# WestlyPark/StyleRenderer

Hardware: AMD Instinct MI355X
Metric: generator fwd+bwd images/sec at 256^2 (higher is better)
Workload: dtype f32

## Files before the change

stylerenderer_amd/build.py:

```python
import os
import subprocess
import sys

HERE = os.path.dirname(os.path.abspath(__file__))
CSRC = os.path.join(HERE, "csrc")
LIB = os.path.join(HERE, "libstylerenderer_hip.so")
OBJ = os.path.join(HERE, "csrc", "_obj")

ARCH = "gfx950"
COMMON = ["--offload-arch=" + ARCH, "-O3", "-std=c++17", "-fPIC", "-Wno-unused-result",
          "-fhip-fp32-correctly-rounded-divide-sqrt"]
EXACT = ["-ffp-contract=off"]
NOSLP = ["-fno-slp-vectorize"]

SOURCES = [
    ("capi.hip", EXACT),
    ("fused_bias_act.hip", EXACT),
    ("upfirdn2d.hip", EXACT + NOSLP),
    ("rasterize.hip", EXACT),
    ("fused_elem.hip", EXACT),
    ("weight_prep.hip", EXACT),
    ("style_linear.hip", EXACT),
    ("bank_mm.hip", EXACT),
    ("mesh.hip", EXACT),
    ("lpips.hip", EXACT),
    ("conv_mfma.hip", []),
    ("conv_wino.hip", []),
    ("conv_wgrad_wino.hip", []),
    ("conv_wgrad_mfma.hip", []),
    ("conv_wgrad_bf16x3.hip", []),
    ("conv_s2_bf16x3.hip", []),
    ("conv_generic.hip", []),
    ("conv1x1_gemm.hip", []),
]


def _hipcc():
    for c in (os.environ.get("HIPCC"), "/opt/rocm/bin/hipcc", "hipcc"):
        if c and (os.path.isabs(c) and os.path.exists(c) or not os.path.isabs(c)):
            return c
    return "hipcc"


def _deps(src):
    deps = [src, os.path.join(CSRC, "common.h"),
            os.path.join(HERE, "..", "include", "stylerenderer_amd.h"), os.path.abspath(__file__)]
    deps += [os.path.join(CSRC, f) for f in os.listdir(CSRC) if f.endswith(".h")]
    return max(os.path.getmtime(d) for d in deps if os.path.exists(d))


def build_library(force=False, verbose=False):
    os.makedirs(OBJ, exist_ok=True)
    hipcc = _hipcc()
    objs, rebuilt = [], False
    procs = []
    for name, extra in SOURCES:
        src = os.path.join(CSRC, name)
        obj = os.path.join(OBJ, name.replace(".hip", ".o"))
        objs.append(obj)
        if force or not os.path.exists(obj) or os.path.getmtime(obj) < _deps(src):
            cmd = [hipcc] + COMMON + extra + ["-c", src, "-o", obj]
            if verbose:
                print(" ".join(cmd))
            procs.append((name, subprocess.Popen(cmd, stdout=subprocess.PIPE, stderr=subprocess.STDOUT)))
            rebuilt = True
    for name, p in procs:
        out, _ = p.communicate()
        if p.returncode != 0:
            sys.stderr.write(out.decode(errors="replace"))
            raise RuntimeError("hipcc failed on %s" % name)
        if verbose and out:
            sys.stdout.write(out.decode(errors="replace"))
    if rebuilt or not os.path.exists(LIB):
        cmd = [hipcc, "--offload-arch=" + ARCH, "-shared", "-fPIC", "-o", LIB] + objs
        if verbose:
            print(" ".join(cmd))
        subprocess.check_call(cmd)
    return LIB


if __name__ == "__main__":
    print(build_library(force="-f" in sys.argv, verbose=True))
```

stylerenderer_amd/csrc/conv_mfma.hip:

```cpp
#include "common.h"
#include "conv1x1_gemm.h"
#include "conv_s2_bf16x3.h"
#include "conv_wgrad_bf16x3.h"
#include "conv_wino.h"

#include <cstdlib>

namespace {

typedef float f32x16 __attribute__((ext_vector_type(16)));
typedef const void __attribute__((address_space(1)))* gptr_t;
typedef void __attribute__((address_space(3)))* lptr_t;

constexpr int BN = 128;
constexpr int BM = 128;

__device__ __attribute__((aligned(16))) const float g_zero_line[4] = {0.f, 0.f, 0.f, 0.f};
__device__ __attribute__((aligned(16))) const float g_ones_line[4] = {1.f, 1.f, 1.f, 1.f};

struct ConvParams {
    const float* in;
    const float* wt;
    const float* iscale;
    const float* oscale;
    const float* obias;
    float* out;
    int B, C, N, ldw;
    int IH, IW;
    int GH, GW;
    int gy_base, gx_base;
    int OH, OW;
    int osy, osx, ooy, oox;
    int dy0, dx0;
    int wmap[9];
    int tiles_x, tiles_y, tiles_b, tiles_n;
    float* partial;
    int64_t partial_floats;
    int ks, c_per_slice;
    int tap_first, tap_step, tap_count;
};

template <int IS, int TY, int TX, int PW, int PH, int PB, bool V4, bool TAP9 = false>
struct Geo {
    static constexpr bool ROT = V4 && IS == 2;
    static constexpr int NT = TY * TX;
    static constexpr int KC = NT >= 9 ? 4 : (NT >= 4 ? 8 : 16);
    static constexpr int EH = (PH - 1) * IS + TY;
    static constexpr int EW = (PW - 1) * IS + TX;
    static constexpr int LEAD = (V4 && !ROT) ? (TAP9 ? 4 : (TX > 1 ? 3 : 0)) : 0;
    static constexpr int EWP = ROT ? (EW + 3 + 3) / 4 * 4
                                   : (V4 ? (LEAD + EW + 3) / 4 * 4 : EW + ((EW % 2 == 0) ? 1 : 0));
    static constexpr int PLANE = PB * EH * EWP;
    static constexpr int W_FLOATS = NT * KC * BN;
    static constexpr int W_INSTR = W_FLOATS / 256;
    static constexpr int IMG_INSTR = V4 ? (KC * PLANE + 255) / 256 : 0;
    static constexpr int ST_INSTR = V4 ? (KC * PB + 63) / 64 : 0;
    static constexpr int IN_FLOATS = KC * PLANE + KC * PB;
    static constexpr int IN_INSTR = V4 ? IMG_INSTR + ST_INSTR : (IN_FLOATS + 63) / 64;
    static constexpr int S_BASE = V4 ? W_FLOATS + IMG_INSTR * 256 : W_FLOATS + KC * PLANE;
    static constexpr int BUF = V4 ? S_BASE + ST_INSTR * 64 : W_FLOATS + IN_INSTR * 64;
    static constexpr int W_PER_WAVE = (W_INSTR + 3) / 4;
    static constexpr int IN_PER_WAVE = (IN_INSTR + 3) / 4;
    static constexpr int LDS_BYTES = 2 * BUF * 4;
};

template <int IS, int TY, int TX, int PW, int PH, int PB, bool V4, bool FAST, bool TAP9 = false>
__global__ __launch_bounds__(256) void k_conv_mfma(const ConvParams p) {
    using G = Geo<IS, TY, TX, PW, PH, PB, V4, TAP9>;
    static_assert(PW * PH * PB == BM, "patch must hold 128 pixels");
    static_assert(!TAP9 || (IS == 1 && TY == 1 && TX == 1), "tap-split mode is a shifted 1x1 convolution");
    extern __shared__ __attribute__((aligned(16))) float smem[];

    const int nwg = gridDim.x;
    int bid = blockIdx.x;
    {
        const int q = nwg / SR_NUM_XCD, r = nwg % SR_NUM_XCD, xcd = bid % SR_NUM_XCD;
        bid = (xcd < r ? xcd * (q + 1) : r * (q + 1) + (xcd - r) * q) + bid / SR_NUM_XCD;
    }
    int tap = 0, g_dy0 = p.dy0, g_dx0 = p.dx0, g_gh = p.GH, g_gw = p.GW, g_ooy = p.ooy, g_oox = p.oox, g_slab = p.wmap[0];
    int tap_local = 0;
    if (TAP9) {
        tap_local = bid % p.tap_count;
        bid /= p.tap_count;
        tap = p.tap_first + tap_local * p.tap_step;
        const int ky = tap / 3, kx = tap - 3 * ky;
        g_dy0 = -(ky >> 1); g_dx0 = -(kx >> 1);
        g_ooy = ky & 1; g_oox = kx & 1;
        g_gh = min(g_ooy ? p.IH : p.IH + 1, p.GH); g_gw = min(g_oox ? p.IW : p.IW + 1, p.GW);
        g_slab = tap;
    }
    const int n_t = bid % p.tiles_n;
    bid /= p.tiles_n;
    const int tx_i = bid % p.tiles_x;
    bid /= p.tiles_x;
    const int ty_i = bid % p.tiles_y;
    bid /= p.tiles_y;
    const int tb_i = bid % p.tiles_b;
    const int slice = bid / p.tiles_b;
    const int c_beg = slice * p.c_per_slice;
    const int c_end = min(p.C, c_beg + p.c_per_slice);
    const int n0 = n_t * BN, gy0 = p.gy_base + ty_i * PH, gx0 = p.gx_base + tx_i * PW, b0 = tb_i * PB;
    const int iy0 = gy0 * IS + g_dy0, ix0 = gx0 * IS + g_dx0;

    const int tid = threadIdx.x, lane = tid & 63;
    const int wave = __builtin_amdgcn_readfirstlane(tid >> 6);
    const int half = lane >> 5, l31 = lane & 31;
    const int wco = wave & 1, wpx = wave >> 1;

    int a_off[2], b_off[2], s_off[2];
    int b_rot[2][4];
#pragma unroll
    for (int t = 0; t < 2; ++t) {
        a_off[t] = half * BN + wco * 64 + t * 32 + l31;
        const int m = wpx * 64 + t * 32 + l31;
        const int px = m % PW, py = (m / PW) % PH, pb = m / (PW * PH);
        b_off[t] = G::W_FLOATS + half * G::PLANE + (pb * G::EH + py * IS) * G::EWP + px * IS + G::LEAD +
                   ((TAP9 && V4) ? g_dx0 : 0);
        s_off[t] = G::S_BASE + pb * G::KC + half;
        const int l0 = half + iy0 + py * IS + ix0;
#pragma unroll
        for (int k = 0; k < 4; ++k) b_rot[t][k] = b_off[t] + ((l0 + k) & 3);
    }

    int w_src[G::W_PER_WAVE];
    int w_cl[G::W_PER_WAVE];
#pragma unroll
    for (int i = 0; i < G::W_PER_WAVE; ++i) {
        const int j = wave + 4 * i;
        const int row = 2 * j + half;
        const int t = row / G::KC, c = row % G::KC;
        const int col = min(n0 + l31 * 4, p.ldw - 4);
        w_cl[i] = (j < G::W_INSTR) ? c : -1;
        int slab = 0;
#pragma unroll
        for (int k = 0; k < G::NT; ++k)
            if (t == k) slab = p.wmap[k];
        if (TAP9) slab = g_slab;
        w_src[i] = (slab * p.C + c) * p.ldw + col;
    }
    int i_src[G::IN_PER_WAVE];
    int i_cl[G::IN_PER_WAVE];
#pragma unroll
    for (int i = 0; i < G::IN_PER_WAVE; ++i) {
        const int j = wave + 4 * i;
        int src = -1, c = 0, pb = 0;
        if (V4) {
            const int f = (j * 64 + lane) * 4;
            if (j < G::IMG_INSTR && f < G::KC * G::PLANE) {
                c = f / G::PLANE;
                const int q = f % G::PLANE;
                const int cola = q % G::EWP, r = (q / G::EWP) % G::EH;
                pb = q / (G::EWP * G::EH);
                const int gy = iy0 + r;
                int gx = ((TAP9 && V4) ? gx0 : ix0) - G::LEAD + cola;
                bool ok = gy >= 0 && gy < p.IH && b0 + pb < p.B;
                if (G::ROT) {
                    gx = ix0 - ((c * (p.IH * p.IW) + gy * p.IW + ix0) & 3) + cola;
                } else {
                    ok = ok && gx >= 0 && gx + 3 < p.IW;
                }
                if (ok) src = (pb * p.C + c) * p.IH * p.IW + gy * p.IW + gx;
            } else if (j >= G::IMG_INSTR && j < G::IN_INSTR) {
                const int e = (j - G::IMG_INSTR) * 64 + lane;
                if (e < G::KC * PB) {
                    pb = e / G::KC;
                    c = e % G::KC;
                    src = -2;
                }
            }
        } else {
            const int f = j * 64 + lane;
            if (j < G::IN_INSTR && f < G::KC * G::PLANE) {
                c = f / G::PLANE;
                const int q = f % G::PLANE;
                const int colp = q % G::EWP, r = (q / G::EWP) % G::EH;
                pb = q / (G::EWP * G::EH);
                const int gy = iy0 + r, gx = ix0 + colp;
                if (colp < G::EW && gy >= 0 && gy < p.IH && gx >= 0 && gx < p.IW && b0 + pb < p.B)
                    src = (pb * p.C + c) * p.IH * p.IW + gy * p.IW + gx;
            } else if (j < G::IN_INSTR && f < G::IN_FLOATS) {
                const int e = f - G::KC * G::PLANE;
                pb = e / G::KC;
                c = e % G::KC;
                src = -2;
            }
        }
        i_src[i] = src;
        i_cl[i] = c | (pb << 8);
    }
    const float* in_base = p.in + (int64_t)b0 * p.C * p.IH * p.IW;
    const int plane_in = p.IH * p.IW;

    const char* f_wp[G::W_PER_WAVE];
    const char* f_ip[G::IN_PER_WAVE];
    unsigned f_is[G::IN_PER_WAVE];
    if (FAST) {
#pragma unroll
        for (int i = 0; i < G::W_PER_WAVE; ++i) f_wp[i] = reinterpret_cast<const char*>(p.wt + w_src[i]);
#pragma unroll
        for (int i = 0; i < G::IN_PER_WAVE; ++i) {
            const int c = i_cl[i] & 255, pb = i_cl[i] >> 8;
            const char* ptr = reinterpret_cast<const char*>(g_zero_line);
            unsigned str = 0;
            if (i_src[i] >= 0) {
                ptr = reinterpret_cast<const char*>(in_base + i_src[i]);
                str = (unsigned)plane_in * 4u;
            } else if (i_src[i] == -2) {
                const bool ok = p.iscale && b0 + pb < p.B;
                ptr = ok ? reinterpret_cast<const char*>(p.iscale + (int64_t)(b0 + pb) * p.C + c)
                         : reinterpret_cast<const char*>(g_ones_line);
                str = ok ? 4u : 0u;
            }
            f_ip[i] = ptr;
            f_is[i] = str;
        }
    }
    const unsigned w_chunk_stride = (unsigned)p.ldw * 4u;

    auto dma = [&](int c0, int buf) {
        float* dst = smem + buf * G::BUF;
        if (FAST) {
#pragma unroll
            for (int i = 0; i < G::W_PER_WAVE; ++i) {
                const int j = wave + 4 * i;
                if (j < G::W_INSTR)
                    __builtin_amdgcn_global_load_lds((gptr_t)(f_wp[i] + (uint64_t)(unsigned)c0 * w_chunk_stride),
                                                     (lptr_t)(dst + j * 256), 16, 0, 0);
            }
#pragma unroll
            for (int i = 0; i < G::IN_PER_WAVE; ++i) {
                const int j = wave + 4 * i;
                if (j < G::IN_INSTR) {
                    const char* src = f_ip[i] + (uint64_t)(unsigned)c0 * f_is[i];
                    if (V4 && j < G::IMG_INSTR)
                        __builtin_amdgcn_global_load_lds((gptr_t)src, (lptr_t)(dst + G::W_FLOATS + j * 256), 16, 0, 0);
                    else if (V4)
                        __builtin_amdgcn_global_load_lds((gptr_t)src,
                                                         (lptr_t)(dst + G::S_BASE + (j - G::IMG_INSTR) * 64), 4, 0, 0);
                    else
                        __builtin_amdgcn_global_load_lds((gptr_t)src, (lptr_t)(dst + G::W_FLOATS + j * 64), 4, 0, 0);
                }
            }
            return;
        }
#pragma unroll
        for (int i = 0; i < G::W_PER_WAVE; ++i) {
            const int j = wave + 4 * i;
            if (j < G::W_INSTR) {
                const float* src = (c0 + w_cl[i] < p.C) ? p.wt + w_src[i] + (int64_t)c0 * p.ldw : g_zero_line;
                __builtin_amdgcn_global_load_lds((gptr_t)src, (lptr_t)(dst + j * 256), 16, 0, 0);
            }
        }
#pragma unroll
        for (int i = 0; i < G::IN_PER_WAVE; ++i) {
            const int j = wave + 4 * i;
            if (j < G::IN_INSTR) {
                const int c = i_cl[i] & 255, pb = i_cl[i] >> 8;
                const bool c_ok = c0 + c < p.C;
                const float* src = g_zero_line;
                if (i_src[i] >= 0 && c_ok) src = in_base + i_src[i] + (int64_t)c0 * plane_in;
                if (i_src[i] == -2)
                    src = (p.iscale && c_ok && b0 + pb < p.B) ? p.iscale + (int64_t)(b0 + pb) * p.C + c0 + c
                                                              : g_ones_line;
                if (V4 && j < G::IMG_INSTR)
                    __builtin_amdgcn_global_load_lds((gptr_t)src, (lptr_t)(dst + G::W_FLOATS + j * 256), 16, 0, 0);
                else if (V4)
                    __builtin_amdgcn_global_load_lds((gptr_t)src,
                                                     (lptr_t)(dst + G::S_BASE + (j - G::IMG_INSTR) * 64), 4, 0, 0);
                else
                    __builtin_amdgcn_global_load_lds((gptr_t)src, (lptr_t)(dst + G::W_FLOATS + j * 64), 4, 0, 0);
            }
        }
    };

    f32x16 acc[2][2];
#pragma unroll
    for (int i = 0; i < 2; ++i)
#pragma unroll
        for (int j = 0; j < 2; ++j)
#pragma unroll
            for (int r = 0; r < 16; ++r) acc[i][j][r] = 0.0f;

    dma(c_beg, 0);
    int buf = 0;
    for (int c0 = c_beg; c0 < c_end; c0 += G::KC) {
        __syncthreads();
        if (c0 + G::KC < c_end) dma(c0 + G::KC, buf ^ 1);
        const float* sb = smem + buf * G::BUF;
#pragma unroll
        for (int cp = 0; cp < G::KC / 2; ++cp) {
            const float sc0 = sb[s_off[0] + 2 * cp];
            const float sc1 = (PB > 1) ? sb[s_off[1] + 2 * cp] : sc0;
#pragma unroll
            for (int ty = 0; ty < TY; ++ty)
#pragma unroll
                for (int tx = 0; tx < TX; ++tx) {
                    const int w_tap = ((ty * TX + tx) * G::KC + 2 * cp) * BN;
                    const int i_tap = (2 * cp) * G::PLANE + ty * G::EWP + tx;
                    float a0 = sb[w_tap + a_off[0]];
                    float a1 = sb[w_tap + a_off[1]];
                    float x0 = sb[i_tap + (G::ROT ? b_rot[0][(2 * cp + ty) & 3] : b_off[0])];
                    float x1 = sb[i_tap + (G::ROT ? b_rot[1][(2 * cp + ty) & 3] : b_off[1])];
                    if (PB == 1) { a0 *= sc0; a1 *= sc0; }
                    else { x0 *= sc0; x1 *= sc1; }
                    acc[0][0] = __builtin_amdgcn_mfma_f32_32x32x2f32(a0, x0, acc[0][0], 0, 0, 0);
                    acc[0][1] = __builtin_amdgcn_mfma_f32_32x32x2f32(a0, x1, acc[0][1], 0, 0, 0);
                    acc[1][0] = __builtin_amdgcn_mfma_f32_32x32x2f32(a1, x0, acc[1][0], 0, 0, 0);
// ... 418 lines not shown
        per = (per + 15) / 16 * 16;
        if (per < 64) per = 64;
        if (per > C) per = C;
        c_per_slice = per;
        ks = (C + per - 1) / per;
        return;
    }
    int pw, ph, pb;
    patch_shape(IW + 1, pw, ph, pb);
    const int64_t blocks = (int64_t)((IW + pw) / pw) * ((IH + ph) / ph) * ((B + pb - 1) / pb) * ((N + BN - 1) / BN) * 9;
    ks = 1;
    c_per_slice = (C + 15) / 16 * 16;
    if (blocks >= 2 * SR_NUM_CU || C < 64) return;
    int want = (int)((2 * SR_NUM_CU + blocks - 1) / blocks);
    if (want > 8) want = 8;
    int per = (C + want - 1) / want;
    per = (per + 15) / 16 * 16;
    if (per < 32) per = 32;
    c_per_slice = per;
    ks = (C + per - 1) / per;
}

int64_t convt_taps_floats(int64_t B, int64_t C, int64_t N, int64_t IH, int64_t IW) {
    int ks, per;
    convt_taps_plan((int)IH, (int)IW, (int)B, (int)N, (int)C, ks, per);
    return (int64_t)ks * 9 * B * N * (IH + 1) * (IW + 1);
}

bool convt_taps_wanted(int64_t B, int64_t C, int64_t N, int64_t IH, int64_t IW) {
    const int mode = convt_taps_mode();
    return mode == 1 || (mode == 2 && 18.0 * (double)B * (double)C * (double)N * (double)IH * (double)IW < 1.05e10);
}

bool taps_v4(const ConvParams& p) {
    const char* e = std::getenv("SR_CONVT_TAPS_V4");
    return !(e && e[0] == '0') && p.IW % 4 == 0 && p.gx_base % 4 == 0 && (reinterpret_cast<uintptr_t>(p.in) & 15) == 0;
}

int launch_convt_taps(ConvParams p, hipStream_t st) {
    p.GH = p.IH + 1; p.GW = p.IW + 1;
    p.gy_base = p.gx_base = 0;
    p.osy = p.osx = 2; p.ooy = p.oox = 0;
    p.dy0 = p.dx0 = 0;
    p.tap_first = 0; p.tap_step = 1; p.tap_count = 9;
    convt_taps_plan(p.IH, p.IW, p.B, p.N, p.C, p.ks, p.c_per_slice);
    int pw, ph, pb;
    patch_shape(p.GW, pw, ph, pb);
    p.tiles_x = (p.GW + pw - 1) / pw;
    p.tiles_y = (p.GH + ph - 1) / ph;
    p.tiles_b = (p.B + pb - 1) / pb;
    p.tiles_n = (p.N + BN - 1) / BN;
    const int64_t blocks = (int64_t)p.tiles_x * p.tiles_y * p.tiles_b * p.tiles_n * p.ks * 9;
    if (blocks > 0x7FFFFFFFLL) return SR_ERANGE;
    const dim3 grid((unsigned)blocks);
    const bool v4 = taps_v4(p);
    int rc;
    if (sr_convt_taps_gemm_eligible(p.B, p.C, p.N, p.IW, p.ldw, p.c_per_slice, p.wt))
        rc = sr_convt_taps_gemm_launch(p.partial, p.in, p.wt, p.ldw, p.iscale, p.B, p.C, p.N, p.IH, p.IW, p.ks, p.c_per_slice, st);
    else if (pw == 32) rc = v4 ? launch_one<1, 1, 1, 32, 4, 1, true, true>(p, grid, st)
                          : launch_one<1, 1, 1, 32, 4, 1, false, true>(p, grid, st);
    else if (pw == 16) rc = v4 ? launch_one<1, 1, 1, 16, 8, 1, true, true>(p, grid, st)
                               : launch_one<1, 1, 1, 16, 8, 1, false, true>(p, grid, st);
    else if (pw == 8) rc = launch_one<1, 1, 1, 8, 8, 2, false, true>(p, grid, st);
    else rc = launch_one<1, 1, 1, 4, 4, 8, false, true>(p, grid, st);
    if (rc != SR_OK) return rc;
    const int64_t total = (int64_t)p.B * p.N * p.OH * p.OW;
    hipLaunchKernelGGL(k_convt_tap_reduce, dim3(sr_stream_grid(total, 256)), dim3(256), 0, st, p);
    return sr_launch_status();
}

__global__ __launch_bounds__(256) void k_convt_strip_reduce(const ConvParams p, const float* __restrict__ prow,
                                                            const float* __restrict__ pcol, int ks_row, int ks_col) {
    const int rw = p.IW + 1, ch = p.IH, OW = p.OW, OH = p.OH;
    const int per_row = OW + OH - 1;
    const int64_t planes = (int64_t)p.B * p.N, total = planes * per_row;
    for (int64_t i = (int64_t)blockIdx.x * blockDim.x + threadIdx.x; i < total;
         i += (int64_t)gridDim.x * blockDim.x) {
        const int64_t row = i / per_row;
        const int q = (int)(i - row * per_row);
        float acc;
        int64_t o;
        acc = 0.0f;
        if (q < OW) {
            const int g = q >> 1;
            const float* t = prow + row * rw + g;
            for (int s = 0; s < ks_row; ++s, t += 3 * planes * rw)
                acc += (q & 1) ? t[planes * rw] : t[0] + t[2 * planes * rw];
            o = (int64_t)(OH - 1) * OW + q;
        } else {
            const int Y = q - OW, g = Y >> 1;
            const float* t = pcol + row * ch + g;
            for (int s = 0; s < ks_col; ++s, t += 3 * planes * ch)
                acc += (Y & 1) ? t[planes * ch] : t[0] + t[2 * planes * ch];
            o = (int64_t)Y * OW + (OW - 1);
        }
        if (p.oscale) acc *= p.oscale[row];
        if (p.obias) acc += p.obias[row % p.N];
        p.out[row * (int64_t)OH * OW + o] = acc;
    }
}

constexpr int STRIP_KS = 4;
int64_t convt_strip_floats(int64_t B, int64_t N, int64_t IH, int64_t IW) { return STRIP_KS * 3 * B * N * (IW + 1 + IH); }

template <int PW, int PH, int PB>
int launch_strip_part(ConvParams& p, hipStream_t st) {
    p.tiles_x = (p.GW - p.gx_base + PW - 1) / PW;
    p.tiles_y = (p.GH - p.gy_base + PH - 1) / PH;
    p.tiles_b = (p.B + PB - 1) / PB;
    p.tiles_n = (p.N + BN - 1) / BN;
    int64_t blocks = (int64_t)p.tiles_x * p.tiles_y * p.tiles_b * p.tiles_n * p.tap_count;
    p.ks = 1; p.c_per_slice = (p.C + 15) / 16 * 16;
    for (int ks = STRIP_KS; ks >= 2; ks /= 2)
        if (p.C % (16 * ks) == 0 && p.C / ks >= 64 && blocks * ks <= 4 * SR_NUM_CU) {
            p.ks = ks;
            p.c_per_slice = p.C / ks;
            break;
        }
    blocks *= p.ks;
    if (blocks > 0x7FFFFFFFLL) return SR_ERANGE;
    if (PB == 1 && taps_v4(p)) return launch_one<1, 1, 1, PW, PH, PB, PB == 1, true>(p, dim3((unsigned)blocks), st);
    return launch_one<1, 1, 1, PW, PH, PB, false, true>(p, dim3((unsigned)blocks), st);
}

int launch_convt_strips(ConvParams p, hipStream_t st) {
    float* prow = p.partial;
    float* pcol = p.partial + STRIP_KS * 3 * (int64_t)p.B * p.N * (p.IW + 1);
    p.osy = p.osx = 2; p.ooy = p.oox = 0;
    p.dy0 = p.dx0 = 0;
    p.ks = 1; p.c_per_slice = (p.C + 15) / 16 * 16;
    p.gy_base = p.IH; p.GH = p.IH + 1; p.gx_base = 0; p.GW = p.IW + 1;
    p.tap_first = 6; p.tap_step = 1; p.tap_count = 3;
    p.partial = prow;
    int rc = launch_strip_part<32, 4, 1>(p, st);
    if (rc != SR_OK) return rc;
    const int ks_row = p.ks;
    p.gy_base = 0; p.GH = p.IH; p.gx_base = p.IW; p.GW = p.IW + 1;
    p.tap_first = 2; p.tap_step = 3; p.tap_count = 3;
    p.partial = pcol;
    rc = launch_strip_part<4, 4, 8>(p, st);
    if (rc != SR_OK) return rc;
    const int ks_col = p.ks;
    const int64_t total = (int64_t)p.B * p.N * (p.OW + p.OH - 1);
    hipLaunchKernelGGL(k_convt_strip_reduce, dim3(sr_stream_grid(total, 256)), dim3(256), 0, st, p, prow, pcol, ks_row,
                       ks_col);
    return sr_launch_status();
}

bool wino_enabled() {
    const char* e = std::getenv("SR_WINOGRAD");
    return !(e && e[0] == '0');
}

bool rot_enabled() {
    const char* e = std::getenv("SR_CONV_ROT");
    return !(e && e[0] == '0');
}

template <int IS, int TY, int TX>
int launch_by_patch(ConvParams& p, hipStream_t st) {
    int pw, ph, pb;
    const int ext_w = p.GW - p.gx_base, ext_h = p.GH - p.gy_base;
    if (ext_w <= 0 || ext_h <= 0) return SR_OK;
    choose_split(ext_h, ext_w, p.B, p.N, p.C, p.ks, p.c_per_slice);
    if (!p.partial || (int64_t)p.ks * p.B * p.N * ext_h * ext_w > p.partial_floats) {
        p.ks = 1;
        p.c_per_slice = (p.C + 15) / 16 * 16;
    }
    patch_shape(ext_w, pw, ph, pb);
    p.tiles_x = (ext_w + pw - 1) / pw;
    p.tiles_y = (ext_h + ph - 1) / ph;
    p.tiles_b = (p.B + pb - 1) / pb;
    p.tiles_n = (p.N + BN - 1) / BN;
    const int64_t blocks = (int64_t)p.tiles_x * p.tiles_y * p.tiles_b * p.tiles_n * p.ks;
    if (blocks <= 0) return SR_OK;
    if (blocks > 0x7FFFFFFFLL) return SR_ERANGE;
    const dim3 grid((unsigned)blocks);
    const bool v4 = IS == 1 && pb == 1 && p.IW % 4 == 0 && (reinterpret_cast<uintptr_t>(p.in) & 15) == 0 &&
                    p.gx_base % 4 == 0 && p.dx0 == (TX > 1 ? -1 : 0);
    const bool rot = IS == 2 && pb == 1 && (p.IW & 3) == 1 && ((p.IH * p.IW) & 3) == 1 && p.C % 4 == 0 &&
                     (reinterpret_cast<uintptr_t>(p.in) & 15) == 0 && p.dx0 >= 0 && p.dy0 >= 0 && p.gx_base == 0 &&
                     p.gy_base == 0 && (p.GW - 1) * 2 + p.dx0 + TX <= p.IW && (p.GH - 1) * 2 + p.dy0 + TY <= p.IH &&
                     ext_w % pw == 0 && ext_h % ph == 0 && rot_enabled();
    int rc;
    if (IS == 1 && v4) {
        if (pw == 32) rc = launch_one<1, TY, TX, 32, 4, 1, true>(p, grid, st);
        else rc = launch_one<1, TY, TX, 16, 8, 1, true>(p, grid, st);
    } else if (IS == 2 && rot && TY == 3 && TX == 3) {
        if (pw == 32) rc = launch_one<2, 3, 3, 32, 4, 1, true>(p, grid, st);
        else rc = launch_one<2, 3, 3, 16, 8, 1, true>(p, grid, st);
    } else if (pw == 32) rc = launch_one<IS, TY, TX, 32, 4, 1, false>(p, grid, st);
    else if (pw == 16) rc = launch_one<IS, TY, TX, 16, 8, 1, false>(p, grid, st);
    else if (pw == 8) rc = launch_one<IS, TY, TX, 8, 8, 2, false>(p, grid, st);
    else rc = launch_one<IS, TY, TX, 4, 4, 8, false>(p, grid, st);
    if (rc != SR_OK || p.ks <= 1) return rc;
    const int64_t total = (int64_t)p.B * p.N * ext_h * ext_w;
    hipLaunchKernelGGL(k_conv_reduce, dim3(sr_stream_grid(total, 256)), dim3(256), 0, st, p, ext_h, ext_w);
    return sr_launch_status();
}

}

extern "C" int64_t sr_conv2d_scratch_floats(int64_t B, int64_t C, int64_t N, int64_t IH, int64_t IW,
                                            int64_t OH, int64_t OW, int ksize, int stride, int pad,
                                            int transposed) {
    (void)ksize; (void)stride; (void)pad;
    if (B <= 0 || C <= 0 || N <= 0 || OH <= 0 || OW <= 0) return 0;
    int ks, per;
    int64_t need = 0;
    auto consider = [&](int64_t gh, int64_t gw) {
        if (gh <= 0 || gw <= 0) return;
        choose_split((int)gh, (int)gw, (int)B, (int)N, (int)C, ks, per);
        if (ks > 1) need = need > ks * B * N * gh * gw ? need : ks * B * N * gh * gw;
    };
    if (!transposed) {
        consider(OH, OW);
        if (ksize == 3 && stride == 2 && pad == 0 && sr_wgrad_bf16x3_enabled('c') &&
            sr_conv_s2_bf16x3_eligible(B, C, N, IH, IW, OH, OW)) {
            const int64_t w = sr_conv_s2_bf16x3_scratch_floats(C, N);
            need = need > w ? need : w;
        }
        if (ksize == 3 && stride == 1 && pad == 1 && wino_enabled() &&
            sr_wino_eligible(B, C, N, IH, IW, nullptr, nullptr)) {
            const int64_t w = sr_wino_scratch_floats(C, N) + sr_wino_partial_floats(B, C, N, IH, IW);
            need = need > w ? need : w;
        }
    } else {
        consider(IH + 1, IW + 1);
        consider(IH, IW);
        consider(1, IW + 1);
        consider(IH, 1);
        if (ksize == 3 && stride == 2 && pad == 0 && convt_taps_wanted(B, C, N, IH, IW)) {
            const int64_t w = convt_taps_floats(B, C, N, IH, IW);
            need = need > w ? need : w;
        }
        if (ksize == 3 && stride == 2 && pad == 0) {
            const int64_t w = convt_strip_floats(B, N, IH, IW), f = convt_fused_split_floats(B, C, N, IH, IW);
            need = need > w ? need : w;
            need = need > f ? need : f;
        }
        if (ksize == 3 && stride == 2 && pad == 0 && sr_wgrad_bf16x3_enabled('t') && sr_convt_bf16x3_eligible(B, C, N, IH, IW)) {
            const int64_t w = sr_convt_bf16x3_scratch_floats(C, N);
            need = need > w ? need : w;
        }
    }
    return need;
}

extern "C" int sr_conv2d_uses_winograd(int64_t B, int64_t C, int64_t N, int64_t IH, int64_t IW, const float* in,
                                       const float* out) {
    return (wino_enabled() && sr_wino_eligible(B, C, N, IH, IW, in, out)) ? 1 : 0;
}

extern "C" int sr_conv2d_mfma_ex(float* out, const float* in, const float* wt, const float* iscale,
                              const float* oscale, const float* obias, int64_t B, int64_t C,
                              int64_t N, int64_t wt_ld, int64_t IH, int64_t IW, int64_t OH, int64_t OW,
                              int ksize, int stride, int pad, int transposed, int flags, float* scratch,
                              sr_stream_t stream) {
    if (B < 0 || C <= 0 || N <= 0 || IH <= 0 || IW <= 0 || OH <= 0 || OW <= 0) return SR_EINVAL;
    if (wt_ld < N || wt_ld % 4 != 0 || (reinterpret_cast<uintptr_t>(wt) & 15)) return SR_EINVAL;
    if (B == 0) return SR_OK;
    if (!out || !in || !wt) return SR_EINVAL;
    if (B * C * IH * IW >= (1LL << 31) || B * N * OH * OW >= (1LL << 40) ||
        (int64_t)ksize * ksize * C * wt_ld >= (1LL << 31))
        return SR_ERANGE;
    hipStream_t st = sr_stream(stream);
    ConvParams p;
    p.in = in; p.wt = wt; p.iscale = iscale; p.oscale = oscale; p.obias = obias; p.out = out;
    p.B = (int)B; p.C = (int)C; p.N = (int)N; p.ldw = (int)wt_ld;
    p.IH = (int)IH; p.IW = (int)IW; p.OH = (int)OH; p.OW = (int)OW;
    p.partial = scratch;
    p.partial_floats = scratch ? sr_conv2d_scratch_floats(B, C, N, IH, IW, OH, OW, ksize, stride, pad, transposed) : 0;
    for (int i = 0; i < 9; ++i) p.wmap[i] = 0;
    p.ks = 1; p.c_per_slice = (p.C + 15) / 16 * 16;
    p.tap_first = 0; p.tap_step = 1; p.tap_count = 9;
    if (!transposed) {
        if (OH != (IH + 2 * pad - ksize) / stride + 1 || OW != (IW + 2 * pad - ksize) / stride + 1)
            return SR_EINVAL;
        p.GH = p.OH; p.GW = p.OW;
        p.gy_base = p.gx_base = 0;
        p.osy = p.osx = 1; p.ooy = p.oox = 0;
        p.dy0 = p.dx0 = -pad;
        for (int i = 0; i < ksize * ksize; ++i) p.wmap[i] = i;
        int rc;
        if (ksize == 3 && stride == 1 && pad == 1 && scratch && wino_enabled() &&
            sr_wino_eligible(B, C, N, IH, IW, in, out))
            return sr_wino_conv3x3(out, in, wt, wt_ld, iscale, oscale, obias, B, C, N, IH, IW, scratch, st, nullptr,
                                   (flags & SR_CONV_U_READY) != 0);
        if (ksize == 3 && stride == 2 && pad == 0 && scratch && sr_wgrad_bf16x3_enabled('c') &&
            sr_conv_s2_bf16x3_eligible(B, C, N, IH, IW, OH, OW))
            return sr_conv_s2_bf16x3_launch(out, in, wt, wt_ld, iscale, oscale, obias, B, C, N, IH, IW, OH, OW, scratch, st);
        if (ksize == 3 && stride == 1) rc = launch_by_patch<1, 3, 3>(p, st);
        else if (ksize == 3 && stride == 2) rc = launch_by_patch<2, 3, 3>(p, st);
        else if (ksize == 1 && stride == 1) {
            if (pad == 0 && sr_conv1x1_gemm_eligible(B, C, N, wt_ld, IH * IW, in, wt, out))
                return sr_conv1x1_gemm_launch(out, in, wt, wt_ld, iscale, oscale, obias, B, C, N, IH * IW, st);
            rc = launch_by_patch<1, 1, 1>(p, st);
        }
        else if (ksize == 1 && stride == 2) rc = launch_by_patch<2, 1, 1>(p, st);
        else return SR_EINVAL;
        return rc;
    }
    if (ksize != 3 || stride != 2 || pad != 0 || OH != 2 * IH + 1 || OW != 2 * IW + 1) return SR_EINVAL;
    if (scratch && convt_taps_wanted(B, C, N, IH, IW) && convt_taps_floats(B, C, N, IH, IW) <= p.partial_floats &&
        !(sr_wgrad_bf16x3_enabled('t') && sr_convt_bf16x3_eligible(B, C, N, IH, IW)))
        return launch_convt_taps(p, st);
    bool fused_ok = false;
    {
        const char* e = std::getenv("SR_CONVT_FUSED");
        const int64_t fused_blocks = (int64_t)(p.IW / TFused::PW) * (p.IH / TFused::PH) * ((p.N + BN - 1) / BN) * p.B;
        bool fused_pays = fused_blocks >= 192 || p.C <= 256;
        if (!fused_pays && scratch && !(e && e[0] == '0')) {
            const char* k = std::getenv("SR_CONVT_FUSED_KS");
            const int ks = (k && k[0] == '0') ? 1 : convt_fused_slices(fused_blocks, p.C);
            if (ks > 1 && convt_fused_eligible(p) && (int64_t)ks * B * N * OH * OW <= p.partial_floats) {
                p.ks = ks;
                p.c_per_slice = p.C / ks;
                fused_pays = true;
            }
        }
        if (scratch && sr_wgrad_bf16x3_enabled('t') && sr_convt_bf16x3_eligible(B, C, N, IH, IW)) {
            const int rc = sr_convt_bf16x3_launch(out, in, wt, wt_ld, iscale, oscale, obias, B, C, N, IH, IW, scratch, st);
            if (rc != SR_OK) return rc;
            fused_ok = true;
        } else if (!(e && e[0] == '0') && p.IW >= 16 && convt_fused_eligible(p) && (fused_pays || (e && e[0] == '1'))) {
            for (int i = 0; i < 9; ++i) p.wmap[i] = i;
            const int rc = launch_convt_fused(p, st);
            p.ks = 1; p.c_per_slice = (p.C + 15) / 16 * 16;
            if (rc != SR_OK) return rc;
            fused_ok = true;
        }
    }
    if (fused_ok && scratch && convt_strip_floats(B, N, IH, IW) <= p.partial_floats) {
        const char* e = std::getenv("SR_CONVT_STRIPS");
        if (!(e && e[0] == '0')) return launch_convt_strips(p, st);
    }
    for (int py = 0; py < 2; ++py)
        for (int px = 0; px < 2; ++px) {
            const int TYp = py == 0 ? 2 : 1, TXp = px == 0 ? 2 : 1;
            p.osy = p.osx = 2; p.ooy = py; p.oox = px;
            p.dy0 = -(TYp - 1); p.dx0 = -(TXp - 1);
            for (int ty = 0; ty < TYp; ++ty)
                for (int tx = 0; tx < TXp; ++tx) {
                    const int ky = py + 2 * (TYp - 1 - ty), kx = px + 2 * (TXp - 1 - tx);
                    p.wmap[ty * TXp + tx] = ky * 3 + kx;
                }
            const int gh_full = py == 0 ? p.IH + 1 : p.IH, gw_full = px == 0 ? p.IW + 1 : p.IW;
            int regions[3][4] = {{0, p.IH, 0, p.IW},
                                 {p.IH, gh_full, 0, gw_full},
                                 {0, p.IH, p.IW, gw_full}};
            const bool split_border = p.IW >= 16;
            if (!split_border) {
                regions[0][1] = gh_full;
                regions[0][3] = gw_full;
            }
            const bool fused = split_border && fused_ok;
            for (int rg = fused ? 1 : 0; rg < (split_border ? 3 : 1); ++rg) {
                p.gy_base = regions[rg][0]; p.GH = regions[rg][1];
                p.gx_base = regions[rg][2]; p.GW = regions[rg][3];
                if (p.GH <= p.gy_base || p.GW <= p.gx_base) continue;
                int rc;
                if (py == 0 && px == 0) rc = launch_by_patch<1, 2, 2>(p, st);
                else if (py == 0) rc = launch_by_patch<1, 2, 1>(p, st);
                else if (px == 0) rc = launch_by_patch<1, 1, 2>(p, st);
                else rc = launch_by_patch<1, 1, 1>(p, st);
                if (rc != SR_OK) return rc;
            }
        }
    return SR_OK;
}

extern "C" int sr_conv2d_mfma(float* out, const float* in, const float* wt, const float* iscale,
                              const float* oscale, const float* obias, int64_t B, int64_t C,
                              int64_t N, int64_t wt_ld, int64_t IH, int64_t IW, int64_t OH, int64_t OW,
                              int ksize, int stride, int pad, int transposed, float* scratch,
                              sr_stream_t stream) {
    return sr_conv2d_mfma_ex(out, in, wt, iscale, oscale, obias, B, C, N, wt_ld, IH, IW, OH, OW, ksize, stride, pad,
                             transposed, 0, scratch, stream);
}

extern "C" int sr_conv2d_nba_ex(float* out, const float* in, const float* wt, const float* iscale, const float* oscale,
                                const float* noise, const float* noise_w, const float* abias, float alpha, float gain,
                                int64_t B, int64_t C, int64_t N, int64_t wt_ld, int64_t H, int64_t W,
                                int64_t noise_bstride, int flags, float* scratch, sr_stream_t stream) {
    if (B < 0 || C <= 0 || N <= 0 || H <= 0 || W <= 0) return SR_EINVAL;
    if (wt_ld < N || wt_ld % 4 != 0 || (reinterpret_cast<uintptr_t>(wt) & 15)) return SR_EINVAL;
    if (B == 0) return SR_OK;
    if (!out || !in || !wt || !scratch || (noise && !noise_w)) return SR_EINVAL;
    if (!wino_enabled() || !sr_wino_eligible(B, C, N, H, W, in, out)) return SR_EINVAL;
    const WinoNba nba{noise, noise_w, abias, noise_bstride, alpha, gain};
    return sr_wino_conv3x3(out, in, wt, wt_ld, iscale, oscale, nullptr, B, C, N, H, W, scratch, sr_stream(stream), &nba,
                           (flags & SR_CONV_U_READY) != 0);
}

extern "C" int sr_conv2d_nba(float* out, const float* in, const float* wt, const float* iscale, const float* oscale,
                             const float* noise, const float* noise_w, const float* abias, float alpha, float gain,
                             int64_t B, int64_t C, int64_t N, int64_t wt_ld, int64_t H, int64_t W,
                             int64_t noise_bstride, float* scratch, sr_stream_t stream) {
    return sr_conv2d_nba_ex(out, in, wt, iscale, oscale, noise, noise_w, abias, alpha, gain, B, C, N, wt_ld, H, W,
                            noise_bstride, 0, scratch, stream);
}
```

Baseline: 552.2.

## Add Winograd-style kernel for stride-2 3x3 transposed convolution

```diff
diff --git a/stylerenderer_amd/build.py b/stylerenderer_amd/build.py
--- a/stylerenderer_amd/build.py
+++ b/stylerenderer_amd/build.py
@@ -30,6 +30,7 @@
     ("conv_wgrad_mfma.hip", []),
     ("conv_wgrad_bf16x3.hip", []),
     ("conv_s2_bf16x3.hip", []),
+    ("conv_s2_wino.hip", []),
     ("conv_generic.hip", []),
     ("conv1x1_gemm.hip", []),
 ]
diff --git a/stylerenderer_amd/csrc/conv_mfma.hip b/stylerenderer_amd/csrc/conv_mfma.hip
--- a/stylerenderer_amd/csrc/conv_mfma.hip
+++ b/stylerenderer_amd/csrc/conv_mfma.hip
@@ -3,6 +3,7 @@
 #include "conv_s2_bf16x3.h"
 #include "conv_wgrad_bf16x3.h"
 #include "conv_wino.h"
+#include "conv_s2_wino.h"
 
 #include <cstdlib>
 
@@ -1027,11 +1028,17 @@
         return rc;
     }
     if (ksize != 3 || stride != 2 || pad != 0 || OH != 2 * IH + 1 || OW != 2 * IW + 1) return SR_EINVAL;
-    if (scratch && convt_taps_wanted(B, C, N, IH, IW) && convt_taps_floats(B, C, N, IH, IW) <= p.partial_floats &&
-        !(sr_wgrad_bf16x3_enabled('t') && sr_convt_bf16x3_eligible(B, C, N, IH, IW)))
+    const bool split_bf16 = sr_wgrad_bf16x3_enabled('t') && sr_convt_bf16x3_eligible(B, C, N, IH, IW);
+    bool fused_ok = false;
+    if (!split_bf16 && sr_convt_wino_enabled() && sr_convt_wino_eligible(B, C, N, wt_ld, IH, IW, in)) {
+        const int rc = sr_convt_wino_launch(out, in, wt, wt_ld, iscale, oscale, obias, B, C, N, IH, IW, st);
+        if (rc != SR_OK) return rc;
+        fused_ok = true;
+    }
+    if (!fused_ok && scratch && convt_taps_wanted(B, C, N, IH, IW) &&
+        convt_taps_floats(B, C, N, IH, IW) <= p.partial_floats && !split_bf16)
         return launch_convt_taps(p, st);
-    bool fused_ok = false;
-    {
+    if (!fused_ok) {
         const char* e = std::getenv("SR_CONVT_FUSED");
         const int64_t fused_blocks = (int64_t)(p.IW / TFused::PW) * (p.IH / TFused::PH) * ((p.N + BN - 1) / BN) * p.B;
         bool fused_pays = fused_blocks >= 192 || p.C <= 256;
diff --git a/stylerenderer_amd/csrc/conv_s2_wino.h b/stylerenderer_amd/csrc/conv_s2_wino.h
--- /dev/null
+++ b/stylerenderer_amd/csrc/conv_s2_wino.h
@@ -0,0 +1,9 @@
+#pragma once
+#include <hip/hip_runtime.h>
+#include <stdint.h>
+
+bool sr_convt_wino_enabled();
+bool sr_convt_wino_eligible(int64_t B, int64_t C, int64_t N, int64_t ldw, int64_t IH, int64_t IW, const void* in);
+int sr_convt_wino_launch(float* out, const float* in, const float* wt, int64_t ldw, const float* iscale,
+                         const float* oscale, const float* obias, int64_t B, int64_t C, int64_t N, int64_t IH,
+                         int64_t IW, hipStream_t st);
diff --git a/stylerenderer_amd/csrc/conv_s2_wino.hip b/stylerenderer_amd/csrc/conv_s2_wino.hip
--- /dev/null
+++ b/stylerenderer_amd/csrc/conv_s2_wino.hip
@@ -0,0 +1,324 @@
+#include "common.h"
+#include "conv_s2_wino.h"
+
+#include <cstdlib>
+
+namespace {
+
+typedef float f32x16 __attribute__((ext_vector_type(16)));
+typedef void __attribute__((address_space(3)))* lptr_t;
+
+template <int CPW>
+struct TW {
+    static constexpr int KC = 8;
+    static constexpr int NB = 64;
+    static constexpr int RPW = 32 / CPW;
+    static constexpr int PH = 2 * RPW, PW = 2 * CPW;
+    static constexpr int LEAD = 3;
+    static constexpr int EWP = PW + 4;
+    static constexpr int EH = PH + 1;
+    static constexpr int PLANE = EH * EWP;
+    static constexpr int W_FLOATS = 9 * KC * NB;
+    static constexpr int W_INSTR = W_FLOATS / 256;
+    static constexpr int I_INSTR = (KC * PLANE / 4 + 63) / 64;
+    static constexpr int BUF = W_FLOATS + I_INSTR * 256;
+    static constexpr int W_PER_WAVE = (W_INSTR + 3) / 4, I_PER_WAVE = (I_INSTR + 3) / 4;
+    static constexpr int PAD = 2 * BUF;
+    static constexpr int STY = PAD + 4 * 256;
+    static_assert(I_PER_WAVE == 2 && W_PER_WAVE == 5, "DMA slots of the step schedule");
+    static_assert(2 * 3072 <= 2 * BUF, "epilogue exchange fits the chunk buffers");
+};
+
+struct WinoTParams {
+    const float* in;
+    const float* wt;
+    const float* iscale;
+    const float* oscale;
+    const float* obias;
+    float* out;
+    int B, C, N, ldw, IH, IW, OH, OW;
+    int tiles_x, tiles_y, tiles_n;
+};
+
+__host__ __device__ constexpr int wsel(int P) { return P < 3 ? P : 3; }
+__host__ __device__ constexpr int isel(int P) { return P < 3 ? P : (P == 3 ? 1 : 3); }
+
+template <int CPW, int HP>
+__device__ __forceinline__ void convt_wino_body(const WinoTParams& p, float* smem, int bid) {
+#if __HIP_DEVICE_COMPILE__
+    using G = TW<CPW>;
+    constexpr int P0 = HP ? 12 : 0, NP = HP ? 13 : 12;
+    float* const sty = smem + G::STY;
+
+    const int n_t = bid % p.tiles_n;
+    bid /= p.tiles_n;
+    const int tx_i = bid % p.tiles_x;
+    bid /= p.tiles_x;
+    const int ty_i = bid % p.tiles_y;
+    const int b = bid / p.tiles_y;
+    const int n0 = n_t * G::NB, j0 = ty_i * G::PH, i0 = tx_i * G::PW;
+
+    const int tid = threadIdx.x, lane = tid & 63;
+    const int wave = __builtin_amdgcn_readfirstlane(tid >> 6);
+    const int half = lane >> 5, l31 = lane & 31;
+    const int g = wave >> 1;
+    const int rp = l31 / CPW, cq = l31 % CPW;
+
+    constexpr int OOB = 0x7FFFFFF0;
+    int w_off[G::W_PER_WAVE];
+#pragma unroll
+    for (int i = 0; i < G::W_PER_WAVE; ++i) {
+        const int j = wave + 4 * i;
+        const int line = j * 64 + lane;
+        const int row = line >> 4, t = row / G::KC, c = row % G::KC;
+        const int col = min(n0 + (line & 15) * 4, p.ldw - 4);
+        w_off[i] = j < G::W_INSTR ? ((t * p.C + c) * p.ldw + col) * 4 : OOB;
+    }
+    int i_off[G::I_PER_WAVE];
+#pragma unroll
+    for (int i = 0; i < G::I_PER_WAVE; ++i) {
+        const int j = wave + 4 * i;
+        const int f = (j * 64 + lane) * 4;
+        int off = OOB;
+        if (j < G::I_INSTR && f < G::KC * G::PLANE) {
+            const int c = f / G::PLANE, q = f % G::PLANE;
+            const int r = q / G::EWP, cola = q % G::EWP;
+            const int gy = j0 - 1 + r, gx = i0 - 4 + cola;
+            if (gy >= 0 && gy < p.IH && gx >= 0 && gx + 3 < p.IW) off = ((c * p.IH + gy) * p.IW + gx) * 4;
+        }
+        i_off[i] = off;
+    }
+    const int plane_in = p.IH * p.IW;
+    const __amdgpu_buffer_rsrc_t r_w = uniform_rsrc(p.wt, 9 * p.C * p.ldw * 4);
+    const __amdgpu_buffer_rsrc_t r_in = uniform_rsrc(p.in + (int64_t)b * p.C * plane_in, p.C * plane_in * 4);
+    const int nchunks = p.C / G::KC;
+
+    auto dma1 = [&](int k, int i) {
+        if (k >= nchunks) return;
+        const int c0 = k * G::KC;
+        float* dst = smem + (k & 1) * G::BUF;
+        if (i < G::I_PER_WAVE) {
+            const int j = wave + 4 * i;
+            __builtin_amdgcn_raw_ptr_buffer_load_lds(
+                r_in, (lptr_t)(j < G::I_INSTR ? dst + G::W_FLOATS + j * 256 : smem + G::PAD + wave * 256), 16, i_off[i],
+                c0 * plane_in * 4, 0, 0);
+        } else {
+            const int ii = i - G::I_PER_WAVE, j = wave + 4 * ii;
+            __builtin_amdgcn_raw_ptr_buffer_load_lds(r_w, (lptr_t)(j < G::W_INSTR ? dst + j * 256 : smem + G::PAD + wave * 256),
+                                                     16, w_off[ii], c0 * p.ldw * 4, 0, 0);
+        }
+    };
+    constexpr int N_DMA = G::W_PER_WAVE + G::I_PER_WAVE;
+
+    f32x16 acc[NP];
+#pragma unroll
+    for (int q = 0; q < NP; ++q)
+#pragma unroll
+        for (int r = 0; r < 16; ++r) acc[q][r] = 0.0f;
+
+    const int a_rd = half * G::NB + g * 32 + l31;
+    const int b_rd = G::W_FLOATS + half * G::PLANE + (2 * rp) * G::EWP + G::LEAD + 2 * cq;
+    float wr[9], xr[9];
+    auto fetch = [&](const float* sb, int cp) {
+#pragma unroll
+        for (int t = 0; t < 9; ++t) wr[t] = sb[(t * G::KC + 2 * cp) * G::NB + a_rd];
+#pragma unroll
+        for (int a = 0; a < 3; ++a)
+#pragma unroll
+            for (int c = 0; c < 3; ++c) xr[a * 3 + c] = sb[2 * cp * G::PLANE + b_rd + a * G::EWP + c];
+    };
+    float U[2][4][4], V[2][4][4];
+    auto xform_w = [&](int set) {
+        float gx[3][4];
+#pragma unroll
+        for (int ky = 0; ky < 3; ++ky) {
+            gx[ky][0] = wr[ky * 3 + 2];
+            gx[ky][1] = wr[ky * 3 + 0] + wr[ky * 3 + 2];
+            gx[ky][2] = wr[ky * 3 + 0];
+            gx[ky][3] = wr[ky * 3 + 1];
+        }
+#pragma unroll
+        for (int x = 0; x < 4; ++x) {
+            U[set][0][x] = gx[2][x];
+            U[set][1][x] = gx[0][x] + gx[2][x];
+            U[set][2][x] = gx[0][x];
+            U[set][3][x] = gx[1][x];
+        }
+    };
+    auto xform_x = [&](int set, float s) {
+        float h[3][4];
+#pragma unroll
+        for (int a = 0; a < 3; ++a) {
+            const float x0 = xr[a * 3] * s, x1 = xr[a * 3 + 1] * s, x2 = xr[a * 3 + 2] * s;
+            h[a][0] = x0 - x1;
+            h[a][1] = x1;
+            h[a][2] = x2 - x1;
+            h[a][3] = x2;
+        }
+#pragma unroll
+        for (int x = 0; x < 4; ++x) {
+            V[set][0][x] = h[0][x] - h[1][x];
+            V[set][1][x] = h[1][x];
+            V[set][2][x] = h[2][x] - h[1][x];
+            V[set][3][x] = h[2][x];
+        }
+    };
+
+#pragma unroll
+    for (int i = 0; i < N_DMA; ++i) dma1(0, i);
+#pragma unroll
+    for (int i = 0; i < 4; ++i) dma1(1, i);
+    for (int c = tid; c < p.C; c += 256) sty[c] = p.iscale ? p.iscale[(int64_t)b * p.C + c] : 1.0f;
+    __builtin_amdgcn_s_waitcnt(0x0F70);
+    __syncthreads();
+    fetch(smem, 0);
+    xform_w(0);
+    xform_x(0, sty[half]);
+
+    for (int k = 0; k < nchunks; ++k) {
+        const float* sb = smem + (k & 1) * G::BUF;
+        const float* sbn = smem + ((k + 1) & 1) * G::BUF;
+#pragma unroll
+        for (int cp = 0; cp < G::KC / 2; ++cp) {
+            const int cur = cp & 1, nxt = cur ^ 1;
+            float s_next;
+            if (cp == G::KC / 2 - 1) {
+                __builtin_amdgcn_s_waitcnt(0x0F70);
+                __syncthreads();
+                fetch(sbn, 0);
+                s_next = sty[min(k + 1, nchunks - 1) * G::KC + half];
+            } else {
+                fetch(sb, cp + 1);
+                s_next = sty[k * G::KC + 2 * (cp + 1) + half];
+            }
+            __builtin_amdgcn_sched_barrier(0);
+#pragma unroll
+            for (int q = 0; q < NP; ++q) {
+                const int pos = P0 + q, py = pos / 5, px = pos % 5;
+                acc[q] = __builtin_amdgcn_mfma_f32_32x32x2f32(U[cur][wsel(py)][wsel(px)], V[cur][isel(py)][isel(px)],
+                                                              acc[q], 0, 0, 0);
+                if (q == 4) xform_w(nxt);
+                if (q == 7) xform_x(nxt, s_next);
+                if ((q & 1) == 1 && q < 8) {
+                    const int u = q >> 1;
+                    if (cp == 0 && u < N_DMA - 4) dma1(k + 1, 4 + u);
+                    else if (cp == G::KC / 2 - 1) dma1(k + 2, u);
+                }
+                __builtin_amdgcn_sched_barrier(0);
+            }
+        }
+    }
+    __builtin_amdgcn_s_waitcnt(0x0F70);
+    __syncthreads();
+
+    float* const xch = smem + g * 3072;
+    if (HP == 1) {
+#pragma unroll
+        for (int q = 0; q < 3; ++q)
+#pragma unroll
+            for (int r = 0; r < 16; ++r) xch[(q * 16 + r) * 64 + lane] = acc[q][r];
+    }
+    __syncthreads();
+    const int64_t plane_out = (int64_t)p.OH * p.OW;
+    const int j = j0 + 2 * rp, i = i0 + 2 * cq;
+#pragma unroll
+    for (int r = 0; r < 16; ++r) {
+        const int n = n0 + g * 32 + (r & 3) + 8 * (r >> 2) + 4 * half;
+        float z[5][5];
+#pragma unroll
+        for (int q = 0; q < NP; ++q) z[(P0 + q) / 5][(P0 + q) % 5] = acc[q][r];
+        if (HP == 0) {
+            z[2][2] = xch[r * 64 + lane];
+            z[2][3] = xch[(16 + r) * 64 + lane];
+            z[2][4] = xch[(32 + r) * 64 + lane];
+        }
+        const float os = p.oscale ? p.oscale[(int64_t)b * p.N + min(n, p.N - 1)] : 1.0f;
+        const float ob = p.obias ? p.obias[min(n, p.N - 1)] : 0.0f;
+        float* o = p.out + ((int64_t)b * p.N + n) * plane_out + (int64_t)(2 * j) * p.OW + 2 * i;
+        auto row4 = [&](float* dst, const float* zr) {
+            dst[0] = (zr[0] + zr[1]) * os + ob;
+            dst[1] = zr[3] * os + ob;
+            dst[2] = (zr[1] + zr[2]) * os + ob;
+            dst[3] = zr[4] * os + ob;
+        };
+        if (n < p.N) {
+            if (HP == 0) {
+                float e0[5], e1[5];
+#pragma unroll
+                for (int x = 0; x < 5; ++x) {
+                    e0[x] = z[0][x] + z[1][x];
+                    e1[x] = z[1][x] + z[2][x];
+                }
+                row4(o, e0);
+                row4(o + 2 * p.OW, e1);
+            } else {
+                row4(o + p.OW, z[3]);
+                row4(o + 3 * p.OW, z[4]);
+            }
+        }
+    }
+#endif
+}
+
+template <int CPW>
+__global__ __launch_bounds__(256) void k_convt_wino(const WinoTParams p) {
+#if __HIP_DEVICE_COMPILE__
+    extern __shared__ __attribute__((aligned(16))) float smem[];
+    const int nwg = gridDim.x;
+    int bid = blockIdx.x;
+    {
+        const int q = nwg / SR_NUM_XCD, r = nwg % SR_NUM_XCD, xcd = bid % SR_NUM_XCD;
+        bid = (xcd < r ? xcd * (q + 1) : r * (q + 1) + (xcd - r) * q) + bid / SR_NUM_XCD;
+    }
+    if ((__builtin_amdgcn_readfirstlane(threadIdx.x >> 6) & 1) == 0) convt_wino_body<CPW, 0>(p, smem, bid);
+    else convt_wino_body<CPW, 1>(p, smem, bid);
+#endif
+}
+
+int pick_cpw(int64_t IH, int64_t IW) {
+    if (IW % 64 == 0 && IH % 2 == 0) return 32;
+    if (IW % 32 == 0 && IH % 4 == 0) return 16;
+    return 0;
+}
+
+int64_t wino_blocks(int cpw, int64_t B, int64_t N, int64_t IH, int64_t IW) {
+    return (IW / (2 * cpw)) * (IH / (64 / cpw)) * ((N + 63) / 64) * B;
+}
+
+}
+
+bool sr_convt_wino_enabled() {
+    const char* e = std::getenv("SR_S2_WINO");
+    return !(e && e[0] == '0');
+}
+
+bool sr_convt_wino_eligible(int64_t B, int64_t C, int64_t N, int64_t ldw, int64_t IH, int64_t IW, const void* in) {
+    const int cpw = pick_cpw(IH, IW);
+    if (!cpw || C % 8 != 0 || C > 2048 || ldw < 4 || (reinterpret_cast<uintptr_t>(in) & 15)) return false;
+    if (C * IH * IW >= (1LL << 29) - 4 || 9LL * C * ldw >= (1LL << 29) - 4) return false;
+    return wino_blocks(cpw, B, N, IH, IW) >= 512;
+}
+
+int sr_convt_wino_launch(float* out, const float* in, const float* wt, int64_t ldw, const float* iscale,
+                         const float* oscale, const float* obias, int64_t B, int64_t C, int64_t N, int64_t IH,
+                         int64_t IW, hipStream_t st) {
+    const int cpw = pick_cpw(IH, IW);
+    if (!cpw) return SR_EINVAL;
+    WinoTParams p;
+    p.in = in; p.wt = wt; p.iscale = iscale; p.oscale = oscale; p.obias = obias; p.out = out;
+    p.B = (int)B; p.C = (int)C; p.N = (int)N; p.ldw = (int)ldw;
+    p.IH = (int)IH; p.IW = (int)IW; p.OH = (int)(2 * IH + 1); p.OW = (int)(2 * IW + 1);
+    p.tiles_x = (int)(IW / (2 * cpw));
+    p.tiles_y = (int)(IH / (64 / cpw));
+    p.tiles_n = (int)((N + 63) / 64);
+    const int64_t blocks = wino_blocks(cpw, B, N, IH, IW);
+    if (blocks > 0x7FFFFFFFLL) return SR_ERANGE;
+    if (cpw == 32) {
+        const int lds = (TW<32>::STY + p.C) * 4;
+        hipLaunchKernelGGL(k_convt_wino<32>, dim3((unsigned)blocks), dim3(256), lds, st, p);
+    } else {
+        const int lds = (TW<16>::STY + p.C) * 4;
+        hipLaunchKernelGGL(k_convt_wino<16>, dim3((unsigned)blocks), dim3(256), lds, st, p);
+    }
+    return sr_launch_status();
+}
```

After: 560.2 (median of 6 runs). 1.5% higher.
